# daigo0927/tf-raft

Hardware: NVIDIA B200
Metric: frame-pairs/sec at 448×512 iters=12; final-flow max-abs vs ref (higher is better)
Workload: dtype f32

## Files before the change

tf_raft_b200/csrc/conv_tc.cuh:

```cuda
#pragma once
#include <stdlib.h>

#include "common.cuh"
#include "tmap.cuh"

namespace raft {

enum TcEpilogue : int {
  EPI_LINEAR = 0,
  EPI_GRU_ZR = 1,
  EPI_GRU_Q = 2,
};
enum TcAct : int { ACT_NONE = 0, ACT_RELU = 1 };

constexpr int kEpiWarpsConv = 16;
constexpr int kTileM = 128;
constexpr int kChunkK = 64;
constexpr int kABytes = kTileM * kChunkK * 2;
constexpr int kEpiPatchBytes = 16 * 2048;
constexpr int kSmemBudget = 227 * 1024 - 2048;
constexpr int kARow3Pixels = 136;
constexpr int kARow3Bytes = 2 * kARow3Pixels * kChunkK * 2;

struct alignas(64) TcConvParams {
  CUtensorMap a_map[2];
  CUtensorMap b_map;
  int nseg, seg_chunks[2], seg_c0[2];
  int kh, kw, ph, pw;
  int stride;
  int B, H, W, TH, TW, tiles_x, tiles_y;
  int bn, n_total;
  int n_tiles_n;
  int nstages, stage_bytes, tmem_cols;
  int group_chunks;
  int mode, act;
  const float* bias;
  const float* inv_scale;
  float out_scale;
  float* out_f32; int f32_stride, f32_c0;
  __half* out_hi; __half* out_lo; int h_stride, h_c0;
  const float* post_scale;
  const float* post_shift;
  const float* residual; int res_stride, res_c0;
  const float* concat_src; int concat_n;
  float* z; int hid;
  float* h;
  long long* dbg;
  int pdl;
  int row3;
  float* adv_coords;
  float* adv_flow;
  int pair;
};

#if defined(__CUDA_ARCH__)
__device__ __forceinline__ float4 ld4(const float* p) { return *reinterpret_cast<const float4*>(p); }
__device__ __forceinline__ float4 ldg4(const float* p) { return __ldg(reinterpret_cast<const float4*>(p)); }
__device__ __forceinline__ void st4(float* p, float4 v) { *reinterpret_cast<float4*>(p) = v; }
__device__ __forceinline__ void st8u(void* p, const uint32_t (&r)[8]) {
#if defined(RAFT_EPI_EXP) && (RAFT_EPI_EXP & 1)
  if (r[0] != 0x7fc12345u) return;
#endif
  asm volatile("st.global.v8.b32 [%0], {%1, %2, %3, %4, %5, %6, %7, %8};" ::"l"(p), "r"(r[0]), "r"(r[1]), "r"(r[2]), "r"(r[3]),
               "r"(r[4]), "r"(r[5]), "r"(r[6]), "r"(r[7])
               : "memory");
}
__device__ __forceinline__ void ldcg8(const float* p, float (&r)[8]) {
#if defined(RAFT_EPI_EXP) && (RAFT_EPI_EXP & 2)
  if (p != nullptr) {
#pragma unroll
    for (int e = 0; e < 8; ++e) r[e] = 0.5f;
    return;
  }
#endif
  asm volatile("ld.global.cg.v8.f32 {%0, %1, %2, %3, %4, %5, %6, %7}, [%8];"
               : "=f"(r[0]), "=f"(r[1]), "=f"(r[2]), "=f"(r[3]), "=f"(r[4]), "=f"(r[5]), "=f"(r[6]), "=f"(r[7])
               : "l"(p));
}
__device__ __forceinline__ void ldnc8(const float* p, float (&r)[8]) {
  asm volatile("ld.global.nc.v8.f32 {%0, %1, %2, %3, %4, %5, %6, %7}, [%8];"
               : "=f"(r[0]), "=f"(r[1]), "=f"(r[2]), "=f"(r[3]), "=f"(r[4]), "=f"(r[5]), "=f"(r[6]), "=f"(r[7])
               : "l"(p));
}
__device__ __forceinline__ void st8f(float* p, float a, float b, float c, float d, float e, float f, float g, float h) {
  const uint32_t r[8] = {__float_as_uint(a), __float_as_uint(b), __float_as_uint(c), __float_as_uint(d),
                         __float_as_uint(e), __float_as_uint(f), __float_as_uint(g), __float_as_uint(h)};
  st8u(p, r);
}
__device__ __forceinline__ float4 ldcg4(const float* p) { return __ldcg(reinterpret_cast<const float4*>(p)); }

#if defined(RAFT_EPI_EXP) && (RAFT_EPI_EXP & 4)
__device__ __forceinline__ float fast_sigmoid(float x) { return x; }
#else
__device__ __forceinline__ float fast_sigmoid(float x) { return __fdividef(1.0f, 1.0f + __expf(-x)); }
#endif
__device__ __forceinline__ float fast_tanh(float x) { return 1.0f - __fdividef(2.0f, 1.0f + __expf(2.0f * x)); }

template <int MODE>
__device__ __forceinline__ void tc_epilogue_regs(const TcConvParams& p, float (&v)[32], size_t pix, int col, int ncol,
                                                 float inv_scale) {
  if (p.bias) {
#pragma unroll
    for (int q = 0; q < 8; ++q) {
      const float4 bq = ldg4(p.bias + col + 4 * q);
      v[4 * q] = v[4 * q] * inv_scale + bq.x; v[4 * q + 1] = v[4 * q + 1] * inv_scale + bq.y;
      v[4 * q + 2] = v[4 * q + 2] * inv_scale + bq.z; v[4 * q + 3] = v[4 * q + 3] * inv_scale + bq.w;
    }
  } else {
#pragma unroll
    for (int j = 0; j < 32; ++j) v[j] *= inv_scale;
  }
  if (MODE == EPI_LINEAR && p.post_scale) {
#pragma unroll
    for (int q = 0; q < 8; ++q) {
      const float4 sc = ldg4(p.post_scale + col + 4 * q), sh = ldg4(p.post_shift + col + 4 * q);
      v[4 * q] = v[4 * q] * sc.x + sh.x; v[4 * q + 1] = v[4 * q + 1] * sc.y + sh.y;
      v[4 * q + 2] = v[4 * q + 2] * sc.z + sh.z; v[4 * q + 3] = v[4 * q + 3] * sc.w + sh.w;
    }
  }

  __half* dhi = nullptr;
// ... 171 lines not shown
    for (int k = 0; k < 4; ++k)
#pragma unroll
      for (int e = 0; e < 4; ++e) v[k][e] *= inv_scale;
  }

  {
    const bool h_vec = ((p.h_stride | p.h_c0) & 3) == 0;
#pragma unroll
    for (int k0 = 0; k0 < 4; k0 += 2) {
      float4 zv[2], hv[2];
#pragma unroll
      for (int kk = 0; kk < 2; ++kk) {
        const bool ok = pixr[k0 + kk] >= 0;
        zv[kk] = ok ? ldcg4(p.z + (size_t)pixr[k0 + kk] * p.hid + col) : make_float4(0.f, 0.f, 0.f, 0.f);
        hv[kk] = ok ? ldcg4(p.h + (size_t)pixr[k0 + kk] * p.hid + col) : make_float4(0.f, 0.f, 0.f, 0.f);
      }
#pragma unroll
      for (int kk = 0; kk < 2; ++kk) {
        const int k = k0 + kk;
        if (pixr[k] < 0) continue;
        v[k][0] = (1.0f - zv[kk].x) * hv[kk].x + zv[kk].x * fast_tanh(v[k][0]);
        v[k][1] = (1.0f - zv[kk].y) * hv[kk].y + zv[kk].y * fast_tanh(v[k][1]);
        v[k][2] = (1.0f - zv[kk].z) * hv[kk].z + zv[kk].z * fast_tanh(v[k][2]);
        v[k][3] = (1.0f - zv[kk].w) * hv[kk].w + zv[kk].w * fast_tanh(v[k][3]);
        st4(p.h + (size_t)pixr[k] * p.hid + col, make_float4(v[k][0], v[k][1], v[k][2], v[k][3]));
        store_split4(p.out_hi, p.out_lo, (size_t)pixr[k] * p.h_stride + p.h_c0 + col, h_vec, v[k]);
      }
    }
  }
}

#endif

template <bool kRowEpi, bool kRow3 = false>
__global__ void __launch_bounds__(64 + 32 * kEpiWarpsConv, 1) conv_tc_kernel(const __grid_constant__ TcConvParams p) {
#if defined(__CUDA_ARCH__)
  constexpr int kEpiWarps = kEpiWarpsConv;
  extern __shared__ uint8_t smem_raw[];
  uint8_t* smem = reinterpret_cast<uint8_t*>((reinterpret_cast<uintptr_t>(smem_raw) + 1023) & ~uintptr_t(1023));
  const int nst = p.nstages;
  const int b_bytes = p.bn * kChunkK * 2;
  uint8_t* stages = smem;
  uint64_t* full_bar = reinterpret_cast<uint64_t*>(stages + (size_t)nst * p.stage_bytes);
  uint64_t* empty_bar = full_bar + nst;
  uint64_t* acc_full = empty_bar + nst;
  uint64_t* acc_empty = acc_full + 2;
  uint32_t* tmem_holder = reinterpret_cast<uint32_t*>(acc_empty + 2);
  float* patches = reinterpret_cast<float*>(stages + (size_t)nst * p.stage_bytes + 256);

  const int warp = threadIdx.x >> 5;
  const int lane = threadIdx.x & 31;

  const int mtiles = p.B * p.tiles_y * p.tiles_x;
  const int ntiles = mtiles * p.n_tiles_n;
  const int ntaps = p.kh * p.kw;
  const int chunks_per_tap = p.seg_chunks[0] + (p.nseg > 1 ? p.seg_chunks[1] : 0);
  const int total = (kRow3 ? p.kh : ntaps) * chunks_per_tap;
  const int gsz = p.group_chunks;
  const int ngroups = (total + gsz - 1) / gsz;
  const int nchunks32 = (p.bn + 31) >> 5;
  constexpr int kParts = kEpiWarps / 4;
  constexpr int kMaxCh = 8 / kParts;
  const int chunks_per_part = (nchunks32 + kParts - 1) / kParts;

  if (warp == 0 && lane == 0) {
    for (int s = 0; s < nst; ++s) {
      mbar_init(&full_bar[s], 1);
      mbar_init(&empty_bar[s], 1);
    }
    for (int i = 0; i < 2; ++i) {
      mbar_init(&acc_full[i], 1);
      mbar_init(&acc_empty[i], 4 * ((nchunks32 + chunks_per_part - 1) / chunks_per_part));
    }
    fence_mbar_init();
    prefetch_tmap(&p.a_map[0]);
    prefetch_tmap(&p.b_map);
    if (p.nseg > 1) prefetch_tmap(&p.a_map[1]);
  }
  if (warp == 1) {
    tmem_alloc(tmem_holder, (uint32_t)p.tmem_cols);
    tmem_relinquish();
  }
  tc_fence_before();
  __syncthreads();
  tc_fence_after();
  const uint32_t tmem_base = *tmem_holder;
  if (p.pdl && warp != 0) {
    asm volatile("griddepcontrol.wait;" ::: "memory");
    asm volatile("griddepcontrol.launch_dependents;" ::: "memory");
  }

  if (warp == 0) {
    if (elect_one()) {
      int it = 0;
      int npre = 0;
      if (p.pdl) {
        if (!kRow3 && (int)blockIdx.x < ntiles) {
          const int n0 = ((int)blockIdx.x / mtiles) * p.bn;
          npre = min(nst, total);
#pragma unroll 1
          for (int i = 0; i < npre; ++i) {
            mbar_arrive_expect_tx(&full_bar[i], (uint32_t)p.stage_bytes);
            tma_load_4d(stages + (size_t)i * p.stage_bytes + 2 * kABytes, &p.b_map, &full_bar[i], (i % chunks_per_tap) * kChunkK,
                        n0, i / chunks_per_tap, 0);
          }
        }
        asm volatile("griddepcontrol.wait;" ::: "memory");
        asm volatile("griddepcontrol.launch_dependents;" ::: "memory");
      }
      for (int t = blockIdx.x; t < ntiles; t += gridDim.x) {
        const int nt = t / mtiles;
        int mt = t - nt * mtiles;
        const int tx = mt % p.tiles_x;
        mt /= p.tiles_x;
        const int ty = mt % p.tiles_y;
        const int b = mt / p.tiles_y;
        const int x0 = tx * p.TW * p.stride, y0 = ty * p.TH * p.stride, n0 = nt * p.bn;
        if constexpr (kRow3) {
          for (int ky = 0; ky < p.kh; ++ky) {
            for (int ch = 0; ch < p.seg_chunks[0]; ++ch, ++it) {
              const int s = it % nst;
              mbar_wait(&empty_bar[s], ((uint32_t)(it / nst) & 1u) ^ 1u);
              if (p.dbg && blockIdx.x == 0 && it < 512) p.dbg[it] = clock64();
              uint8_t* st = stages + (size_t)s * p.stage_bytes;
              mbar_arrive_expect_tx(&full_bar[s], (uint32_t)p.stage_bytes);
              tma_load_5d(st, &p.a_map[0], &full_bar[s], p.seg_c0[0] + ch * kChunkK, x0 - p.pw, y0 + ky - p.ph, b, 0);
              tma_load_4d(st + kARow3Bytes, &p.b_map, &full_bar[s], ch * kChunkK, n0, ky * p.kw, 0);
            }
          }
        } else {
          for (int tap = 0; tap < ntaps; ++tap) {
            const int dy = tap / p.kw - p.ph, dx = tap % p.kw - p.pw;
            int kc = 0;
            for (int seg = 0; seg < p.nseg; ++seg) {
              for (int ch = 0; ch < p.seg_chunks[seg]; ++ch, ++kc, ++it) {
                const int s = it % nst;
                const uint32_t phase = (uint32_t)(it / nst) & 1u;
                mbar_wait(&empty_bar[s], phase ^ 1u);
                if (p.dbg && blockIdx.x == 0 && it < 512) p.dbg[it] = clock64();
                uint8_t* st = stages + (size_t)s * p.stage_bytes;
                const int c = p.seg_c0[seg] + ch * kChunkK;
#if defined(RAFT_TC_EXP) && (RAFT_TC_EXP & 6)
                if (RAFT_TC_EXP & 2) {
                  mbar_arrive_expect_tx(&full_bar[s], (uint32_t)(2 * kABytes));
                  tma_load_5d(st, &p.a_map[seg], &full_bar[s], c, x0 + dx, y0 + dy, b, 0);
                } else {
                  mbar_arrive_expect_tx(&full_bar[s], (uint32_t)(p.stage_bytes - 2 * kABytes));
                  tma_load_4d(st + 2 * kABytes, &p.b_map, &full_bar[s], kc * kChunkK, n0, tap, 0);
                }
#else
                if (it >= npre) mbar_arrive_expect_tx(&full_bar[s], (uint32_t)p.stage_bytes);
                tma_load_5d(st, &p.a_map[seg], &full_bar[s], c, x0 + dx, y0 + dy, b, 0);
                if (it >= npre) tma_load_4d(st + 2 * kABytes, &p.b_map, &full_bar[s], kc * kChunkK, n0, tap, 0);
#endif
              }
            }
          }
        }
      }
    }
  } else if (warp == 1) {
    const uint32_t idesc = make_idesc_f16(kTileM, p.bn);
    int it = 0, gg = 0;
    for (int t = blockIdx.x; t < ntiles; t += gridDim.x) {
      int done = 0;
      for (int g = 0; g < ngroups; ++g, ++gg) {
        const int buf = gg & 1;
        mbar_wait(&acc_empty[buf], ((uint32_t)(gg >> 1) & 1u) ^ 1u);
        tc_fence_after();
        if (p.dbg && blockIdx.x == 0 && gg < 256 && lane == 0) p.dbg[1024 + 256 + gg] = clock64();
        const uint32_t d_tmem = tmem_base + (uint32_t)(buf * p.bn);
        const int gend = min(total, done + gsz);
        for (int first = 1; done < gend; ++done, ++it, first = 0) {
          const int s = it % nst;
          const uint32_t phase = (uint32_t)(it / nst) & 1u;
          mbar_wait(&full_bar[s], phase);
          tc_fence_after();
          if (p.dbg && blockIdx.x == 0 && it < 512 && lane == 0) p.dbg[512 + it] = clock64();
          if (elect_one()) {
            const uint32_t sa = smem_u32(stages + (size_t)s * p.stage_bytes);
            if constexpr (kRow3) {
#pragma unroll 1
              for (int dx = 0; dx < 3; ++dx) {
                const uint64_t a_hi = make_desc_sw128(sa + dx * 128);
                const uint64_t a_lo = make_desc_sw128(sa + kARow3Bytes / 2 + dx * 128);
                const uint64_t b_hi = make_desc_sw128(sa + kARow3Bytes + dx * b_bytes);
                const uint64_t b_lo = make_desc_sw128(sa + kARow3Bytes + (3 + dx) * b_bytes);
                umma_chunk3<false>(d_tmem, a_hi, a_lo, b_hi, b_lo, idesc, first != 0 && dx == 0);
              }
            } else {
              const uint64_t a_hi = make_desc_sw128(sa);
              const uint64_t a_lo = make_desc_sw128(sa + kABytes);
              const uint64_t b_hi = make_desc_sw128(sa + 2 * kABytes);
              const uint64_t b_lo = make_desc_sw128(sa + 2 * kABytes + b_bytes);
#if defined(RAFT_TC_EXP) && (RAFT_TC_EXP & 1)
              if (sa != 0xffffffffu) goto tc_exp_skip_mma;
#endif
              umma_chunk3<false>(d_tmem, a_hi, a_lo, b_hi, b_lo, idesc, first != 0);
#if defined(RAFT_TC_EXP) && (RAFT_TC_EXP & 1)
            tc_exp_skip_mma:;
#endif
            }
            umma_commit(&empty_bar[s]);
            if (done == gend - 1) umma_commit(&acc_full[buf]);
          }
          __syncwarp();
        }
      }
    }
  } else {
    const int quarter = warp & 3;
    const int part_id = (warp - 2) >> 2;
    const int chunk0 = part_id * chunks_per_part;
    const int my_chunks = max(0, min(chunks_per_part, nchunks32 - chunk0));
    const int m = quarter * 32 + lane;
    const int xl = m % p.TW, yl = m / p.TW;
    const float inv_scale = p.inv_scale ? __ldg(p.inv_scale) : 1.0f;
    const uint32_t trow = tmem_base + ((uint32_t)(quarter * 32) << 16);

    if (my_chunks > 0) {
      int gg = 0;
      for (int t = blockIdx.x; t < ntiles; t += gridDim.x) {
        float racc[kMaxCh][32];
#pragma unroll
        for (int ci = 0; ci < kMaxCh; ++ci)
#pragma unroll
          for (int j = 0; j < 32; ++j) racc[ci][j] = 0.0f;

        for (int g = 0; g < ngroups; ++g, ++gg) {
          const int buf = gg & 1;
          mbar_wait(&acc_full[buf], (uint32_t)(gg >> 1) & 1u);
          tc_fence_after();
          if (p.dbg && blockIdx.x == 0 && gg < 256 && warp == 2 && lane == 0) p.dbg[1024 + gg] = clock64();
#pragma unroll
          for (int ci = 0; ci < kMaxCh; ++ci) {
            if (ci < my_chunks) {
              const int c0 = (chunk0 + ci) * 32;
              uint32_t r[32];
              if (p.bn - c0 >= 32) {
                tmem_ld_32x32(trow + (uint32_t)(buf * p.bn + c0), r);
              } else {
                uint32_t r16[16];
// ... 103 lines not shown
  p.tiles_y = ceil_div(p.H, p.TH);
  p.stage_bytes = 2 * kABytes + 2 * (p.pair ? p.bn / 2 : p.bn) * kChunkK * 2;
  if (p.row3) p.stage_bytes = kARow3Bytes + 3 * 2 * p.bn * kChunkK * 2;
  const int patch = tc_uses_patch(p.mode) ? kEpiPatchBytes : 0;
  int nst = (kSmemBudget - patch) / p.stage_bytes;
  if (nst > 8) nst = 8;
  p.nstages = nst;
  int cols = 32;
  while (cols < 2 * p.bn) cols <<= 1;
  p.tmem_cols = cols;
  if (p.group_chunks <= 0) p.group_chunks = 2;
  return nst * p.stage_bytes + 1024  + 256  + patch;
}

inline bool tc_pdl_enabled() {
  static const int pdl = [] { const char* e = getenv("RAFT_B200_PDL"); return e ? atoi(e) : 1; }();
  return pdl != 0;
}

inline int tc_launch(TcConvParams& p, int n_tiles_n, cudaStream_t stream) {
  if (p.bn % 16 != 0 || p.bn < 16 || p.bn > 256 || p.TW * p.TH != kTileM) return RAFT_ERR_BAD_SHAPE;
  if (p.mode != EPI_LINEAR && p.mode != EPI_GRU_ZR && p.mode != EPI_GRU_Q) return RAFT_ERR_UNSUPPORTED;
  if (p.stride < 1) p.stride = 1;
  const int smem = tc_finalize(p);
  if (p.nstages < 2) return RAFT_ERR_UNSUPPORTED;
  int dev = 0;
  RAFT_CUDA_TRY(cudaGetDevice(&dev));
  const unsigned long long dev_bit = 1ull << (dev & 63);
  static unsigned long long attr_set_mask = 0;
  if (!(attr_set_mask & dev_bit)) {
    RAFT_CUDA_TRY(cudaFuncSetAttribute(conv_tc_kernel<false>, cudaFuncAttributeMaxDynamicSharedMemorySize, 227 * 1024));
    RAFT_CUDA_TRY(cudaFuncSetAttribute(conv_tc_kernel<true>, cudaFuncAttributeMaxDynamicSharedMemorySize, 227 * 1024));
    RAFT_CUDA_TRY(cudaFuncSetAttribute(conv_tc_kernel<true, true>, cudaFuncAttributeMaxDynamicSharedMemorySize, 227 * 1024));
    attr_set_mask |= dev_bit;
  }
  const int mtiles = p.B * p.tiles_y * p.tiles_x;
  p.n_tiles_n = n_tiles_n;
  const long ntiles = (long)mtiles * n_tiles_n;
  const unsigned grid = (unsigned)(ntiles < kNumSMs ? ntiles : kNumSMs);
  p.pdl = tc_pdl_enabled() ? 1 : 0;
  const int threads = 64 + 32 * kEpiWarpsConv;
  if (p.row3 && (p.mode != EPI_LINEAR || p.kh != 3 || p.kw != 3 || p.stride != 1 || p.TH != 1 || p.TW != kTileM || p.nseg != 1 ||
                 p.bn % 8 != 0 || n_tiles_n != 1))
    return RAFT_ERR_UNSUPPORTED;
  void (*kern)(TcConvParams) = p.mode == EPI_GRU_Q ? conv_tc_kernel<false> : (p.row3 ? conv_tc_kernel<true, true> : conv_tc_kernel<true>);
  if (!p.pdl) {
    kern<<<grid, threads, smem, stream>>>(p);
  } else {
    cudaLaunchConfig_t cfg;
    memset(&cfg, 0, sizeof(cfg));
    cfg.gridDim = dim3(grid);
    cfg.blockDim = dim3((unsigned)threads);
    cfg.dynamicSmemBytes = (size_t)smem;
    cfg.stream = stream;
    cudaLaunchAttribute attr[1];
    attr[0].id = cudaLaunchAttributeProgrammaticStreamSerialization;
    attr[0].val.programmaticStreamSerializationAllowed = 1;
    cfg.attrs = attr;
    cfg.numAttrs = 1;
    RAFT_CUDA_TRY(cudaLaunchKernelEx(&cfg, kern, p));
  }
  return raft_launch_status();
}

}
```

tf_raft_b200/csrc/encoder.cuh:

```cuda
#pragma once
#include <algorithm>

#include "lookup.cuh"
#include "update.cuh"

namespace raft {

enum { NORM_NONE = 0, NORM_INSTANCE = 1, NORM_BATCH = 2 };

struct EncSpec { int c0; int c[3]; int s[3]; };
inline EncSpec enc_spec(int variant) {
  if (variant == RAFT_VARIANT_BASIC) return {64, {64, 96, 128}, {1, 2, 2}};
  return {32, {32, 64, 96}, {1, 2, 2}};
}
inline int pad64(int c) { return round_up(c, 64); }

struct EncConvSlot { size_t hi, lo, bias, scale, absmax; int kh, kw, cin, cout, cin_pad, cout_pad; };
struct EncNormSlot { size_t gamma, beta, fscale, fshift; int C; };
struct EncLayout {
  EncConvSlot conv1;
  EncNormSlot norm1;
  EncConvSlot bc1[6], bc2[6], bds[6];
  EncNormSlot bn1[6], bn2[6], bnd[6];
  int has_ds[6], bcin[6], bc[6], bstride[6];
// ... 20 lines not shown
  auto norm_slot = [&](int C) {
    EncNormSlot n;
    n.C = C;
    n.gamma = take(sizeof(float) * (C + 64)); n.beta = take(sizeof(float) * (C + 64));
    n.fscale = take(sizeof(float) * (C + 64)); n.fshift = take(sizeof(float) * (C + 64));
    return n;
  };
  L.conv1 = conv_slot(1, 1, 147, S.c0);
  L.norm1 = norm_slot(S.c0);
  int cin = S.c0;
  for (int k = 0; k < 6; ++k) {
    const int c = S.c[k / 2], st = (k % 2 == 0) ? S.s[k / 2] : 1;
    L.bcin[k] = cin; L.bc[k] = c; L.bstride[k] = st;
    L.bc1[k] = conv_slot(3, 3, cin, c);
    L.bc2[k] = conv_slot(3, 3, c, c);
    L.bn1[k] = norm_slot(c);
    L.bn2[k] = norm_slot(c);
    L.has_ds[k] = st != 1;
    if (L.has_ds[k]) { L.bds[k] = conv_slot(1, 1, cin, c); L.bnd[k] = norm_slot(c); }
    cin = c;
  }
  L.conv2 = conv_slot(1, 1, cin, out_dim);
  L.total = off;
  return L;
}

struct EncWs {
  float *X32, *O32, *Y32, *D32;
  __half *Xh, *Xl, *Oh, *Ol, *Fh, *Fl, *Ih, *Il;
  float *part, *mean, *mult;
  size_t total;
};
constexpr int kNormSplit = 64;
inline EncWs enc_ws_layout(void* base, int variant, int N, int H, int W) {
  EncWs E;
  memset(&E, 0, sizeof(E));
  const EncSpec S = enc_spec(variant);
  size_t max32 = 0, max16 = 0;
  for (int l = 0; l < 3; ++l) {
    const int d = 2 << l;
    const size_t np = (size_t)N * ((H + d - 1) / d) * ((W + d - 1) / d);
    const int c = l == 0 ? (S.c0 > S.c[0] ? S.c0 : S.c[0]) : S.c[l];
    if (np * c > max32) max32 = np * c;
    if (np * pad64(c) > max16) max16 = np * pad64(c);
  }
  uint8_t* b8 = reinterpret_cast<uint8_t*>(base);
  size_t off = 0;
  auto take = [&](size_t bytes) { uint8_t* p = b8 + off; off = align_up(off + bytes, 1024); return p; };
  E.X32 = (float*)take(max32 * 4); E.O32 = (float*)take(max32 * 4);
  E.Y32 = (float*)take(max32 * 4); E.D32 = (float*)take(max32 * 4);
  E.Xh = (__half*)take(max16 * 2); E.Xl = (__half*)take(max16 * 2);
  E.Oh = (__half*)take(max16 * 2); E.Ol = (__half*)take(max16 * 2);
  E.Fh = (__half*)take(max16 * 2); E.Fl = (__half*)take(max16 * 2);
  {
    const size_t np1 = (size_t)N * ((H + 1) / 2) * ((W + 1) / 2);
    E.Ih = (__half*)take(np1 * 192 * 2); E.Il = (__half*)take(np1 * 192 * 2);
  }
  E.part = (float*)take((size_t)N * kNormSplit * 3 * 256 * 4);
  E.mean = (float*)take((size_t)N * 256 * 4);
  E.mult = (float*)take((size_t)N * 256 * 4);
  E.total = off;
  return E;
}

inline int enc_pack_conv(const raft_conv& cv, const EncConvSlot& s, uint8_t* base, cudaStream_t st) {
  if (!cv.kernel || !cv.bias) return RAFT_ERR_BAD_ARG;
  if (cv.kh != s.kh || cv.kw != s.kw || cv.cin != s.cin || cv.cout != s.cout) return RAFT_ERR_BAD_SHAPE;
  const size_t nw = (size_t)s.kh * s.kw * s.cin * s.cout;
  unsigned int* amax = reinterpret_cast<unsigned int*>(base + s.absmax);
  float* scale = reinterpret_cast<float*>(base + s.scale);
  absmax_kernel<<<grid_for(nw), 256, 0, st>>>(cv.kernel, nw, amax);
  weight_scale_kernel<<<1, 1, 0, st>>>(amax, scale);
  PackParams pp;
  memset(&pp, 0, sizeof(pp));
  pp.w = cv.kernel; pp.kh = s.kh; pp.kw = s.kw; pp.cin = s.cin; pp.cout = s.cout;
  pp.hi = reinterpret_cast<__half*>(base + s.hi); pp.lo = reinterpret_cast<__half*>(base + s.lo);
  pp.cout_pad = s.cout_pad; pp.cin_pad = s.cin_pad; pp.cout_off = 0;
  pp.nrange = 1; pp.r_src0[0] = 0; pp.r_n[0] = s.cin; pp.r_dst0[0] = 0;
  pp.scale = scale;
  pack_weights_kernel<<<grid_for(nw), 256, 0, st>>>(pp);
  g_launches += 3;
  RAFT_CUDA_TRY(cudaMemcpyAsync(base + s.bias, cv.bias, s.cout * sizeof(float), cudaMemcpyDeviceToDevice, st));
  return raft_launch_status();
}

inline int enc_pack_norm(const raft_norm& nm, const EncNormSlot& s, int norm_type, uint8_t* base, cudaStream_t st) {
  if (norm_type == NORM_NONE) return 0;
  if (!nm.gamma || !nm.beta) return RAFT_ERR_BAD_ARG;
  float* g = reinterpret_cast<float*>(base + s.gamma);
// ... 30 lines not shown
    RAFT_TRY(enc_pack_conv(w->block[k].conv2, L.bc2[k], base, st));
    RAFT_TRY(enc_pack_norm(w->block[k].norm1, L.bn1[k], norm_type, base, st));
    RAFT_TRY(enc_pack_norm(w->block[k].norm2, L.bn2[k], norm_type, base, st));
    if (L.has_ds[k]) {
      RAFT_TRY(enc_pack_conv(w->block[k].downsample, L.bds[k], base, st));
      RAFT_TRY(enc_pack_norm(w->block[k].downsample_norm, L.bnd[k], norm_type, base, st));
    }
  }
  RAFT_TRY(enc_pack_conv(w->conv2, L.conv2, base, st));
  return raft_launch_status();
}

struct EncCtx {
  const uint8_t* prep; EncLayout L; EncWs W; cudaStream_t st;
  int N, norm_type, stats;
  int per_image;
};

inline int enc_norm_apply(const EncCtx& c, const EncNormSlot& ns, const float* y, size_t npix, int P, int relu,
                          const float* skip32, const __half* skip_hi, const __half* skip_lo, float* out32, __half* hi,
                          __half* lo) {
  const int C = ns.C, G = c.per_image ? c.N : 1;
  const int Pg = c.per_image ? P : (int)npix;
  const float* gamma = reinterpret_cast<const float*>(c.prep + ns.gamma);
  const float* beta = reinterpret_cast<const float*>(c.prep + ns.beta);
  norm_stats_kernel<<<dim3((unsigned)G, kNormSplit), 256, 0, c.st>>>(y, Pg, C, kNormSplit, c.W.part);
  norm_final_kernel<<<ceil_div(G * C * 32, 256), 256, 0, c.st>>>(c.W.part, G, C, kNormSplit, gamma, 1e-3f, c.W.mean, c.W.mult);
  norm_apply_kernel<<<grid_for(npix * (pad64(C) / 8)), 256, 0, c.st>>>(y, npix, P, C, c.per_image, c.W.mean, c.W.mult, beta, relu,
                                                                 skip32, skip_hi, skip_lo, out32, hi, lo, pad64(C));
  g_launches += 3;
  return raft_launch_status();
}

inline int enc_conv_tc(const EncCtx& c, const EncConvSlot& cs, const EncNormSlot* ns, const __half* ahi, const __half* alo,
                       int Hin, int Win, int Hout, int Wout, int stride, int relu, const float* skip, float* out32,
                       __half* ohi, __half* olo) {
  TcConvParams p;
  memset(&p, 0, sizeof(p));
  int tw, th;
  tc_pick_tile(Wout, Hout, &tw, &th);
  if (tw * stride > 256) tw = 128 / stride, th = 128 / tw;
  static const int row3_flag = [] { const char* e = getenv("RAFT_B200_ROW3"); return e ? atoi(e) : 1; }();
  const bool row3 = row3_flag && cs.kh == 3 && cs.kw == 3 && stride == 1 && tw == kTileM && th == 1 && cs.cout_pad <= 96 &&
                    cs.cout_pad % 8 == 0;
  if (row3) {
    RAFT_TRY(make_tmap_act2(&p.a_map[0], ahi, alo, c.N, Hin, Win, cs.cin_pad, kARow3Pixels, 1, 1));
    RAFT_TRY(make_tmap_wgt3(&p.b_map, reinterpret_cast<const __half*>(c.prep + cs.hi),
                            reinterpret_cast<const __half*>(c.prep + cs.lo), cs.kh * cs.kw, cs.cout_pad, cs.cin_pad, cs.cout_pad));
    p.row3 = 1;
  } else {
    RAFT_TRY(make_tmap_act2(&p.a_map[0], ahi, alo, c.N, Hin, Win, cs.cin_pad, tw, th, stride));
    RAFT_TRY(make_tmap_wgt2(&p.b_map, reinterpret_cast<const __half*>(c.prep + cs.hi),
                            reinterpret_cast<const __half*>(c.prep + cs.lo), cs.kh * cs.kw, cs.cout_pad, cs.cin_pad,
                            cs.cout_pad));
  }
  p.nseg = 1; p.seg_chunks[0] = cs.cin_pad / kChunkK; p.seg_c0[0] = 0;
  p.kh = cs.kh; p.kw = cs.kw; p.stride = stride;
  if (stride == 1) { p.ph = (cs.kh - 1) / 2; p.pw = (cs.kw - 1) / 2; }
  else {
    const int tot_h = (Hout - 1) * stride + cs.kh - Hin, tot_w = (Wout - 1) * stride + cs.kw - Win;
    p.ph = (tot_h > 0 ? tot_h : 0) / 2; p.pw = (tot_w > 0 ? tot_w : 0) / 2;
  }
  p.B = c.N; p.H = Hout; p.W = Wout; p.TH = th; p.TW = tw;
  p.bn = cs.cout_pad; p.n_total = cs.cout;
  p.mode = EPI_LINEAR; p.out_scale = 1.0f;
  p.bias = reinterpret_cast<const float*>(c.prep + cs.bias);
  p.inv_scale = reinterpret_cast<const float*>(c.prep + cs.scale) + 1;
  p.out_f32 = out32; p.f32_stride = cs.cout; p.f32_c0 = 0;
  p.out_hi = ohi; p.out_lo = olo; p.h_stride = pad64(cs.cout); p.h_c0 = 0;
  if (ns && !c.stats && c.norm_type == NORM_BATCH) {
    p.post_scale = reinterpret_cast<const float*>(c.prep + ns->fscale);
    p.post_shift = reinterpret_cast<const float*>(c.prep + ns->fshift);
  }
  const bool fused = !(ns && c.stats);
  if (fused) {
    p.act = relu ? ACT_RELU : ACT_NONE;
    p.residual = skip; p.res_stride = cs.cout; p.res_c0 = 0;
  } else {
    p.act = ACT_NONE; p.out_hi = nullptr; p.out_lo = nullptr;
  }
  if (g_dbg_layer >= 1000 && g_dbg_count++ == g_dbg_layer - 1000) p.dbg = g_dbg_buf;
  {
    static const int grp = [] { const char* e = getenv("RAFT_B200_ENC_GROUP"); return e ? atoi(e) : 5; }();
    if (grp > 0) p.group_chunks = grp;
    if (row3) p.group_chunks = 2;
  }
  ++g_launches;
  return tc_launch(p, 1, c.st);
}

inline int encoder_forward(int variant, int norm_type, int out_dim, const void* prepared, const float* images, int N,
                           int H, int W, int training, int image_norm, float* out, void* ws, size_t ws_bytes, cudaStream_t st) {
  EncCtx c;
  c.prep = reinterpret_cast<const uint8_t*>(prepared);
  c.L = enc_layout(variant, out_dim);
  c.W = enc_ws_layout(ws, variant, N, H, W);
  if (c.W.total > ws_bytes) return RAFT_ERR_WORKSPACE;
  c.st = st; c.N = N; c.norm_type = norm_type;
  c.stats = (norm_type == NORM_INSTANCE) || (norm_type == NORM_BATCH && training);
  c.per_image = norm_type == NORM_INSTANCE;
  const EncSpec S = enc_spec(variant);
  const EncLayout& L = c.L;
  const EncWs& E = c.W;

  int h = (H + 1) / 2, w = (W + 1) / 2;
  {
    const size_t npix = (size_t)N * h * w;
    const int tot_h = (h - 1) * 2 + 7 - H, tot_w = (w - 1) * 2 + 7 - W;
    const float* src = images;
    if (image_norm) {
      const size_t nimg = (size_t)N * H * W * 3;
      image_norm_kernel<<<grid_for(nimg), 256, 0, st>>>(images, E.O32, nimg);
      ++g_launches;
      src = E.O32;
    }
    stem_im2col_kernel<<<grid_for(npix * 24), 256, 0, st>>>(src, N, H, W, h, w, (tot_h > 0 ? tot_h : 0) / 2,
                                                            (tot_w > 0 ? tot_w : 0) / 2, 0, E.Ih, E.Il);
    ++g_launches;
    if (!c.stats && pad64(S.c0) != S.c0) {
      RAFT_CUDA_TRY(cudaMemsetAsync(E.Xh, 0, npix * pad64(S.c0) * 2, st));
      RAFT_CUDA_TRY(cudaMemsetAsync(E.Xl, 0, npix * pad64(S.c0) * 2, st));
    }
    RAFT_TRY(enc_conv_tc(c, L.conv1, &L.norm1, E.Ih, E.Il, h, w, h, w, 1, 1, nullptr, c.stats ? E.Y32 : E.X32, E.Xh, E.Xl));
    if (c.stats) RAFT_TRY(enc_norm_apply(c, L.norm1, E.Y32, npix, h * w, 1, nullptr, nullptr, nullptr, nullptr, E.Xh, E.Xl));
  }

  float *X32 = E.X32, *O32 = E.O32;
  __half *Xh = E.Xh, *Xl = E.Xl, *Oh = E.Oh, *Ol = E.Ol;
  for (int k = 0; k < 6; ++k) {
    const int st2 = L.bstride[k], cin = L.bcin[k], cc = L.bc[k];
    const int ho = (h + st2 - 1) / st2, wo = (w + st2 - 1) / st2;
    const size_t npo = (size_t)N * ho * wo;
    (void)cin;
    const bool zero_pad_out = pad64(cc) != cc;
    if (!c.stats && zero_pad_out) {
      RAFT_CUDA_TRY(cudaMemsetAsync(E.Fh, 0, npo * pad64(cc) * 2, st));
      RAFT_CUDA_TRY(cudaMemsetAsync(E.Fl, 0, npo * pad64(cc) * 2, st));
      RAFT_CUDA_TRY(cudaMemsetAsync(Oh, 0, npo * pad64(cc) * 2, st));
      RAFT_CUDA_TRY(cudaMemsetAsync(Ol, 0, npo * pad64(cc) * 2, st));
    }
    RAFT_TRY(enc_conv_tc(c, L.bc1[k], &L.bn1[k], Xh, Xl, h, w, ho, wo, st2, 1, nullptr, c.stats ? E.Y32 : nullptr, E.Fh, E.Fl));
    if (c.stats) RAFT_TRY(enc_norm_apply(c, L.bn1[k], E.Y32, npo, ho * wo, 1, nullptr, nullptr, nullptr, nullptr, E.Fh, E.Fl));
    const float* skip = X32;
    if (L.has_ds[k]) {
      RAFT_TRY(enc_conv_tc(c, L.bds[k], &L.bnd[k], Xh, Xl, h, w, ho, wo, st2, 0, nullptr, c.stats ? E.Y32 : E.D32, nullptr, nullptr));
      if (c.stats) RAFT_TRY(enc_norm_apply(c, L.bnd[k], E.Y32, npo, ho * wo, 0, nullptr, nullptr, nullptr, E.D32, nullptr, nullptr));
      skip = E.D32;
    }
    RAFT_TRY(enc_conv_tc(c, L.bc2[k], &L.bn2[k], E.Fh, E.Fl, ho, wo, ho, wo, 1, 1, skip, c.stats ? E.Y32 : O32, Oh, Ol));
    if (c.stats) {
      if (L.has_ds[k]) RAFT_TRY(enc_norm_apply(c, L.bn2[k], E.Y32, npo, ho * wo, 1, E.D32, nullptr, nullptr, nullptr, Oh, Ol));
      else RAFT_TRY(enc_norm_apply(c, L.bn2[k], E.Y32, npo, ho * wo, 1, nullptr, Xh, Xl, nullptr, Oh, Ol));
    }
    float* t32 = X32; X32 = O32; O32 = t32;
    __half* th_ = Xh; Xh = Oh; Oh = th_;
    __half* tl_ = Xl; Xl = Ol; Ol = tl_;
// ... 8 lines not shown
```

tf_raft_b200/csrc/kernels.cuh:

```cuda
#pragma once
#include "common.cuh"

namespace raft {

__global__ void split_plane_kernel(const float* __restrict__ src, int src_stride, int src_c0, int nch, int nch_pad,
                                   __half* __restrict__ hi, __half* __restrict__ lo, int dst_stride, int dst_c0,
                                   size_t npix, float scale) {
  const size_t total = npix * (size_t)nch_pad;
  for (size_t i = blockIdx.x * (size_t)blockDim.x + threadIdx.x; i < total; i += (size_t)gridDim.x * blockDim.x) {
    const size_t px = i / nch_pad;
    const int c = (int)(i - px * nch_pad);
    __half h = __float2half_rn(0.f), l = h;
    if (c < nch) split_f16(src[px * src_stride + src_c0 + c] * scale, h, l);
    hi[px * dst_stride + dst_c0 + c] = h;
    lo[px * dst_stride + dst_c0 + c] = l;
  }
}

__global__ void avgpool2x2_kernel(const float* __restrict__ src, float* __restrict__ dst, size_t M, int H, int W,
                                  int C) {
  const int Ho = H / 2, Wo = W / 2;
  const size_t total = M * (size_t)Ho * Wo * C;
  for (size_t i = blockIdx.x * (size_t)blockDim.x + threadIdx.x; i < total; i += (size_t)gridDim.x * blockDim.x) {
    size_t t = i;
// ... 531 lines not shown
        const float ss[8] = {s0.x, s0.y, s0.z, s0.w, s1.x, s1.y, s1.z, s1.w};
#pragma unroll
        for (int e = 0; e < 8; ++e) v[e] = fmaxf(ss[e] + v[e], 0.f);
      } else if (skip_hi) {
        const uint4 h4 = *reinterpret_cast<const uint4*>(skip_hi + px * c_pad + c), l4 = *reinterpret_cast<const uint4*>(skip_lo + px * c_pad + c);
        const uint32_t hw[4] = {h4.x, h4.y, h4.z, h4.w}, lw[4] = {l4.x, l4.y, l4.z, l4.w};
#pragma unroll
        for (int e = 0; e < 4; ++e) {
          const float2 hf = __half22float2(*reinterpret_cast<const __half2*>(&hw[e]));
          const float2 lf = __half22float2(*reinterpret_cast<const __half2*>(&lw[e]));
          v[2 * e] = fmaxf(hf.x + lf.x + v[2 * e], 0.f);
          v[2 * e + 1] = fmaxf(hf.y + lf.y + v[2 * e + 1], 0.f);
        }
      }
      if (out32) {
        *reinterpret_cast<float4*>(out32 + px * C + c) = make_float4(v[0], v[1], v[2], v[3]);
        *reinterpret_cast<float4*>(out32 + px * C + c + 4) = make_float4(v[4], v[5], v[6], v[7]);
      }
    }
    if (hi) {
      uint32_t ph[4], pl[4];
#pragma unroll
      for (int e = 0; e < 4; ++e) split_f16x2(v[2 * e], v[2 * e + 1], ph[e], pl[e]);
      *reinterpret_cast<uint4*>(hi + px * c_pad + c) = make_uint4(ph[0], ph[1], ph[2], ph[3]);
      *reinterpret_cast<uint4*>(lo + px * c_pad + c) = make_uint4(pl[0], pl[1], pl[2], pl[3]);
    }
  }
}
__global__ void image_norm_kernel(const float* __restrict__ img, float* __restrict__ out, size_t n) {
  for (size_t i = blockIdx.x * (size_t)blockDim.x + threadIdx.x; i < n; i += (size_t)gridDim.x * blockDim.x)
    out[i] = __fsub_rn(__fmul_rn(2.0f, __fdiv_rn(img[i], 255.0f)), 1.0f);
}

__global__ void stem_im2col_kernel(const float* __restrict__ img, int N, int H, int W, int h, int w, int pad_t,
                                   int pad_l, int image_norm, __half* __restrict__ hi, __half* __restrict__ lo) {
  const size_t total = (size_t)N * h * w * 24;
  for (size_t i = blockIdx.x * (size_t)blockDim.x + threadIdx.x; i < total; i += (size_t)gridDim.x * blockDim.x) {
    const int grp = (int)(i % 24);
    const size_t px = i / 24;
    const int x = (int)(px % w), y = (int)((px / w) % h), n = (int)(px / ((size_t)w * h));
    uint32_t ph[4] = {0u, 0u, 0u, 0u}, pl[4] = {0u, 0u, 0u, 0u};
    if (grp * 8 < 147) {
      int ty = (grp * 8) / 21, j = grp * 8 - ty * 21;
      const int ix0 = 2 * x - pad_l;
      const float* base = img + ((size_t)n * H * W + ix0) * 3;
      float v[8];
#pragma unroll
      for (int e = 0; e < 8; ++e) {
        const int iy = 2 * y + ty - pad_t, ix = ix0 + ((j * 11) >> 5);
        v[e] = 0.f;
        if (ty < 7 && iy >= 0 && iy < H && ix >= 0 && ix < W) {
          v[e] = __ldg(base + (ptrdiff_t)iy * W * 3 + j);
          if (image_norm) v[e] = __fsub_rn(__fmul_rn(2.0f, __fdiv_rn(v[e], 255.0f)), 1.0f);
        }
        if (++j == 21) { j = 0; ++ty; }
      }
#pragma unroll
      for (int e = 0; e < 4; ++e) split_f16x2(v[2 * e], v[2 * e + 1], ph[e], pl[e]);
    }
    reinterpret_cast<uint4*>(hi)[i] = make_uint4(ph[0], ph[1], ph[2], ph[3]);
    reinterpret_cast<uint4*>(lo)[i] = make_uint4(pl[0], pl[1], pl[2], pl[3]);
  }
}

__device__ __forceinline__ void flow_im2col_rider(const float* __restrict__ flow, int B, int h, int w, __half* __restrict__ hi,
                                                  __half* __restrict__ lo, size_t tid, size_t nthreads) {
  const size_t total = (size_t)B * h * w * 16;
  for (size_t i = tid; i < total; i += nthreads) {
    const int g = (int)(i & 15);
    const size_t px = i >> 4;
    const int x = (int)(px % w), y = (int)((px / w) % h);
    uint32_t ph[4], pl[4];
#pragma unroll
    for (int e = 0; e < 4; ++e) {
      const int tap = 4 * g + e;
      float2 v = make_float2(0.f, 0.f);
      if (tap < 49) {
        const int yy = y + tap / 7 - 3, xx = x + tap % 7 - 3;
        if (yy >= 0 && yy < h && xx >= 0 && xx < w)
          v = __ldg(reinterpret_cast<const float2*>(flow) + (ptrdiff_t)px + (ptrdiff_t)(yy - y) * w + (xx - x));
      }
      split_f16x2(v.x, v.y, ph[e], pl[e]);
    }
    reinterpret_cast<uint4*>(hi)[i] = make_uint4(ph[0], ph[1], ph[2], ph[3]);
    reinterpret_cast<uint4*>(lo)[i] = make_uint4(pl[0], pl[1], pl[2], pl[3]);
  }
}

__global__ void flow_im2col_kernel(const float* __restrict__ flow, int B, int h, int w, __half* __restrict__ hi,
                                   __half* __restrict__ lo) {
  const size_t total = (size_t)B * h * w * 128;
  for (size_t i = blockIdx.x * (size_t)blockDim.x + threadIdx.x; i < total; i += (size_t)gridDim.x * blockDim.x) {
// ... 47 lines not shown
```

Baseline: 555.2.

## Fuse stem im2col into tensor-core conv via in-kernel gather warps

Adds a gather mode to the tcgen05 conv kernel. Half of the epilogue warps build the 7x7 stride-2 stem im2col A tiles directly in shared memory, with the swizzle and hi/lo fp16 split, and signal the full barrier, while TMA loads only the weights. This removes the separate stem_im2col kernel launch and its large hi/lo global buffer round trip. In exchange the kernel has fewer epilogue warps free for output, and the register-heavy gather may stall the MMA pipeline.

```diff
diff --git a/tf_raft_b200/csrc/conv_tc.cuh b/tf_raft_b200/csrc/conv_tc.cuh
--- a/tf_raft_b200/csrc/conv_tc.cuh
+++ b/tf_raft_b200/csrc/conv_tc.cuh
@@ -2,6 +2,7 @@
 #include <stdlib.h>
 
 #include "common.cuh"
+#include "kernels.cuh"
 #include "tmap.cuh"
 
 namespace raft {
@@ -21,6 +22,8 @@
 constexpr int kSmemBudget = 227 * 1024 - 2048;
 constexpr int kARow3Pixels = 136;
 constexpr int kARow3Bytes = 2 * kARow3Pixels * kChunkK * 2;
+constexpr int kGatherWarps = kEpiWarpsConv / 2;
+constexpr int kGatherWarp0 = 2 + kEpiWarpsConv - kGatherWarps;
 
 struct alignas(64) TcConvParams {
   CUtensorMap a_map[2];
@@ -51,6 +54,8 @@
   float* adv_coords;
   float* adv_flow;
   int pair;
+  int gather;
+  const float* gather_img; int gather_H, gather_W, gather_pad_t, gather_pad_l;
 };
 
 #if defined(__CUDA_ARCH__)
@@ -87,6 +92,9 @@
                          __float_as_uint(e), __float_as_uint(f), __float_as_uint(g), __float_as_uint(h)};
   st8u(p, r);
 }
+__device__ __forceinline__ void sts128(uint32_t addr, const uint32_t (&r)[4]) {
+  asm volatile("st.shared.v4.b32 [%0], {%1, %2, %3, %4};" ::"r"(addr), "r"(r[0]), "r"(r[1]), "r"(r[2]), "r"(r[3]) : "memory");
+}
 __device__ __forceinline__ float4 ldcg4(const float* p) { return __ldcg(reinterpret_cast<const float4*>(p)); }
 
 #if defined(RAFT_EPI_EXP) && (RAFT_EPI_EXP & 4)
@@ -324,7 +332,7 @@
 
 #endif
 
-template <bool kRowEpi, bool kRow3 = false>
+template <bool kRowEpi, bool kRow3 = false, bool kGather = false>
 __global__ void __launch_bounds__(64 + 32 * kEpiWarpsConv, 1) conv_tc_kernel(const __grid_constant__ TcConvParams p) {
 #if defined(__CUDA_ARCH__)
   constexpr int kEpiWarps = kEpiWarpsConv;
@@ -355,9 +363,10 @@
   constexpr int kMaxCh = 8 / kParts;
   const int chunks_per_part = (nchunks32 + kParts - 1) / kParts;
 
+  const uint32_t tx_bytes = (uint32_t)(kGather ? p.stage_bytes - 2 * kABytes : p.stage_bytes);
   if (warp == 0 && lane == 0) {
     for (int s = 0; s < nst; ++s) {
-      mbar_init(&full_bar[s], 1);
+      mbar_init(&full_bar[s], kGather ? 1 + kGatherWarps : 1);
       mbar_init(&empty_bar[s], 1);
     }
     for (int i = 0; i < 2; ++i) {
@@ -365,7 +374,7 @@
       mbar_init(&acc_empty[i], 4 * ((nchunks32 + chunks_per_part - 1) / chunks_per_part));
     }
     fence_mbar_init();
-    prefetch_tmap(&p.a_map[0]);
+    if (!kGather) prefetch_tmap(&p.a_map[0]);
     prefetch_tmap(&p.b_map);
     if (p.nseg > 1) prefetch_tmap(&p.a_map[1]);
   }
@@ -392,7 +401,7 @@
           npre = min(nst, total);
 #pragma unroll 1
           for (int i = 0; i < npre; ++i) {
-            mbar_arrive_expect_tx(&full_bar[i], (uint32_t)p.stage_bytes);
+            mbar_arrive_expect_tx(&full_bar[i], tx_bytes);
             tma_load_4d(stages + (size_t)i * p.stage_bytes + 2 * kABytes, &p.b_map, &full_bar[i], (i % chunks_per_tap) * kChunkK,
                         n0, i / chunks_per_tap, 0);
           }
@@ -441,8 +450,8 @@
                   tma_load_4d(st + 2 * kABytes, &p.b_map, &full_bar[s], kc * kChunkK, n0, tap, 0);
                 }
 #else
-                if (it >= npre) mbar_arrive_expect_tx(&full_bar[s], (uint32_t)p.stage_bytes);
-                tma_load_5d(st, &p.a_map[seg], &full_bar[s], c, x0 + dx, y0 + dy, b, 0);
+                if (it >= npre) mbar_arrive_expect_tx(&full_bar[s], tx_bytes);
+                if (!kGather) tma_load_5d(st, &p.a_map[seg], &full_bar[s], c, x0 + dx, y0 + dy, b, 0);
                 if (it >= npre) tma_load_4d(st + 2 * kABytes, &p.b_map, &full_bar[s], kc * kChunkK, n0, tap, 0);
 #endif
               }
@@ -500,6 +509,57 @@
         }
       }
     }
+  } else if (kGather && warp >= kGatherWarp0) {
+    constexpr int kUnits = 8 * kTileM / (32 * kGatherWarps);
+    constexpr int kStemChunks = kStemKPad / kChunkK;
+    const int gt = (int)threadIdx.x - 32 * kGatherWarp0;
+    const int m = gt & (kTileM - 1);
+    const bool upper = gt >= kTileM;
+    const int xl = m % p.TW, yl = m / p.TW;
+    int it = 0;
+    for (int t = blockIdx.x; t < ntiles; t += gridDim.x) {
+      int mt = t % mtiles;
+      const int tx = mt % p.tiles_x;
+      mt /= p.tiles_x;
+      const int ty = mt % p.tiles_y;
+      const int b = mt / p.tiles_y;
+      const int x = tx * p.TW + xl, y = ty * p.TH + yl;
+      const bool inside = x < p.W && y < p.H;
+#pragma unroll
+      for (int ch = 0; ch < kStemChunks; ++ch, ++it) {
+        const int s = it % nst;
+        float v[kUnits][8];
+#pragma unroll
+        for (int k = 0; k < kUnits; ++k)
+#pragma unroll
+          for (int e = 0; e < 8; ++e) v[k][e] = 0.f;
+        if (inside) {
+          if (upper) {
+#pragma unroll
+            for (int k = 0; k < kUnits; ++k)
+              stem_window8(p.gather_img, p.gather_H, p.gather_W, p.gather_pad_t, p.gather_pad_l, 0, b, y, x, ch * 8 + kUnits + k, v[k]);
+          } else {
+#pragma unroll
+            for (int k = 0; k < kUnits; ++k)
+              stem_window8(p.gather_img, p.gather_H, p.gather_W, p.gather_pad_t, p.gather_pad_l, 0, b, y, x, ch * 8 + k, v[k]);
+          }
+        }
+        mbar_wait(&empty_bar[s], ((uint32_t)(it / nst) & 1u) ^ 1u);
+        const uint32_t sa = smem_u32(stages + (size_t)s * p.stage_bytes) + (uint32_t)(m * 128);
+#pragma unroll
+        for (int k = 0; k < kUnits; ++k) {
+          uint32_t ph[4], pl[4];
+#pragma unroll
+          for (int e = 0; e < 4; ++e) split_f16x2(v[k][2 * e], v[k][2 * e + 1], ph[e], pl[e]);
+          const uint32_t off = (uint32_t)((((upper ? kUnits : 0) + k) ^ (m & 7)) << 4);
+          sts128(sa + off, ph);
+          sts128(sa + kABytes + off, pl);
+        }
+        fence_proxy_async();
+        __syncwarp();
+        if (lane == 0) mbar_arrive(&full_bar[s]);
+      }
+    }
   } else {
     const int quarter = warp & 3;
     const int part_id = (warp - 2) >> 2;
@@ -669,6 +729,7 @@
     RAFT_CUDA_TRY(cudaFuncSetAttribute(conv_tc_kernel<false>, cudaFuncAttributeMaxDynamicSharedMemorySize, 227 * 1024));
     RAFT_CUDA_TRY(cudaFuncSetAttribute(conv_tc_kernel<true>, cudaFuncAttributeMaxDynamicSharedMemorySize, 227 * 1024));
     RAFT_CUDA_TRY(cudaFuncSetAttribute(conv_tc_kernel<true, true>, cudaFuncAttributeMaxDynamicSharedMemorySize, 227 * 1024));
+    RAFT_CUDA_TRY(cudaFuncSetAttribute(conv_tc_kernel<true, false, true>, cudaFuncAttributeMaxDynamicSharedMemorySize, 227 * 1024));
     attr_set_mask |= dev_bit;
   }
   const int mtiles = p.B * p.tiles_y * p.tiles_x;
@@ -680,7 +741,13 @@
   if (p.row3 && (p.mode != EPI_LINEAR || p.kh != 3 || p.kw != 3 || p.stride != 1 || p.TH != 1 || p.TW != kTileM || p.nseg != 1 ||
                  p.bn % 8 != 0 || n_tiles_n != 1))
     return RAFT_ERR_UNSUPPORTED;
-  void (*kern)(TcConvParams) = p.mode == EPI_GRU_Q ? conv_tc_kernel<false> : (p.row3 ? conv_tc_kernel<true, true> : conv_tc_kernel<true>);
+  if (p.gather && (p.mode != EPI_LINEAR || p.kh != 1 || p.kw != 1 || p.stride != 1 || p.row3 || p.nseg != 1 || p.seg_c0[0] != 0 ||
+                   p.seg_chunks[0] * kChunkK != kStemKPad || p.bn > 64 || n_tiles_n != 1 || !p.gather_img))
+    return RAFT_ERR_UNSUPPORTED;
+  void (*kern)(TcConvParams) = p.mode == EPI_GRU_Q ? conv_tc_kernel<false>
+                               : p.row3            ? conv_tc_kernel<true, true>
+                               : p.gather          ? conv_tc_kernel<true, false, true>
+                                                   : conv_tc_kernel<true>;
   if (!p.pdl) {
     kern<<<grid, threads, smem, stream>>>(p);
   } else {
diff --git a/tf_raft_b200/csrc/encoder.cuh b/tf_raft_b200/csrc/encoder.cuh
--- a/tf_raft_b200/csrc/encoder.cuh
+++ b/tf_raft_b200/csrc/encoder.cuh
@@ -76,6 +76,12 @@
   size_t total;
 };
 constexpr int kNormSplit = 64;
+
+inline bool stem_gather_enabled() {
+  static const int v = [] { const char* e = getenv("RAFT_B200_STEM_GATHER"); return e ? atoi(e) : 1; }();
+  return v != 0;
+}
+
 inline EncWs enc_ws_layout(void* base, int variant, int N, int H, int W) {
   EncWs E;
   memset(&E, 0, sizeof(E));
@@ -96,9 +102,9 @@
   E.Xh = (__half*)take(max16 * 2); E.Xl = (__half*)take(max16 * 2);
   E.Oh = (__half*)take(max16 * 2); E.Ol = (__half*)take(max16 * 2);
   E.Fh = (__half*)take(max16 * 2); E.Fl = (__half*)take(max16 * 2);
-  {
+  if (!stem_gather_enabled()) {
     const size_t np1 = (size_t)N * ((H + 1) / 2) * ((W + 1) / 2);
-    E.Ih = (__half*)take(np1 * 192 * 2); E.Il = (__half*)take(np1 * 192 * 2);
+    E.Ih = (__half*)take(np1 * kStemKPad * 2); E.Il = (__half*)take(np1 * kStemKPad * 2);
   }
   E.part = (float*)take((size_t)N * kNormSplit * 3 * 256 * 4);
   E.mean = (float*)take((size_t)N * 256 * 4);
@@ -195,9 +201,11 @@
   return raft_launch_status();
 }
 
+struct StemGather { const float* img; int H, W, pad_t, pad_l; };
+
 inline int enc_conv_tc(const EncCtx& c, const EncConvSlot& cs, const EncNormSlot* ns, const __half* ahi, const __half* alo,
                        int Hin, int Win, int Hout, int Wout, int stride, int relu, const float* skip, float* out32,
-                       __half* ohi, __half* olo) {
+                       __half* ohi, __half* olo, const StemGather* gather = nullptr) {
   TcConvParams p;
   memset(&p, 0, sizeof(p));
   int tw, th;
@@ -206,7 +214,14 @@
   static const int row3_flag = [] { const char* e = getenv("RAFT_B200_ROW3"); return e ? atoi(e) : 1; }();
   const bool row3 = row3_flag && cs.kh == 3 && cs.kw == 3 && stride == 1 && tw == kTileM && th == 1 && cs.cout_pad <= 96 &&
                     cs.cout_pad % 8 == 0;
-  if (row3) {
+  if (gather) {
+    RAFT_TRY(make_tmap_wgt2(&p.b_map, reinterpret_cast<const __half*>(c.prep + cs.hi),
+                            reinterpret_cast<const __half*>(c.prep + cs.lo), cs.kh * cs.kw, cs.cout_pad, cs.cin_pad,
+                            cs.cout_pad));
+    p.gather = 1;
+    p.gather_img = gather->img; p.gather_H = gather->H; p.gather_W = gather->W;
+    p.gather_pad_t = gather->pad_t; p.gather_pad_l = gather->pad_l;
+  } else if (row3) {
     RAFT_TRY(make_tmap_act2(&p.a_map[0], ahi, alo, c.N, Hin, Win, cs.cin_pad, kARow3Pixels, 1, 1));
     RAFT_TRY(make_tmap_wgt3(&p.b_map, reinterpret_cast<const __half*>(c.prep + cs.hi),
                             reinterpret_cast<const __half*>(c.prep + cs.lo), cs.kh * cs.kw, cs.cout_pad, cs.cin_pad, cs.cout_pad));
@@ -270,6 +285,7 @@
   {
     const size_t npix = (size_t)N * h * w;
     const int tot_h = (h - 1) * 2 + 7 - H, tot_w = (w - 1) * 2 + 7 - W;
+    const int pad_t = (tot_h > 0 ? tot_h : 0) / 2, pad_l = (tot_w > 0 ? tot_w : 0) / 2;
     const float* src = images;
     if (image_norm) {
       const size_t nimg = (size_t)N * H * W * 3;
@@ -277,14 +293,18 @@
       ++g_launches;
       src = E.O32;
     }
-    stem_im2col_kernel<<<grid_for(npix * 24), 256, 0, st>>>(src, N, H, W, h, w, (tot_h > 0 ? tot_h : 0) / 2,
-                                                            (tot_w > 0 ? tot_w : 0) / 2, 0, E.Ih, E.Il);
-    ++g_launches;
+    const bool gather = stem_gather_enabled();
+    if (!gather) {
+      stem_im2col_kernel<<<grid_for(npix * (kStemKPad / 8)), 256, 0, st>>>(src, N, H, W, h, w, pad_t, pad_l, 0, E.Ih, E.Il);
+      ++g_launches;
+    }
     if (!c.stats && pad64(S.c0) != S.c0) {
       RAFT_CUDA_TRY(cudaMemsetAsync(E.Xh, 0, npix * pad64(S.c0) * 2, st));
       RAFT_CUDA_TRY(cudaMemsetAsync(E.Xl, 0, npix * pad64(S.c0) * 2, st));
     }
-    RAFT_TRY(enc_conv_tc(c, L.conv1, &L.norm1, E.Ih, E.Il, h, w, h, w, 1, 1, nullptr, c.stats ? E.Y32 : E.X32, E.Xh, E.Xl));
+    const StemGather sg = {src, H, W, pad_t, pad_l};
+    RAFT_TRY(enc_conv_tc(c, L.conv1, &L.norm1, E.Ih, E.Il, h, w, h, w, 1, 1, nullptr, c.stats ? E.Y32 : E.X32, E.Xh, E.Xl,
+                         gather ? &sg : nullptr));
     if (c.stats) RAFT_TRY(enc_norm_apply(c, L.norm1, E.Y32, npix, h * w, 1, nullptr, nullptr, nullptr, nullptr, E.Xh, E.Xl));
   }
 
diff --git a/tf_raft_b200/csrc/kernels.cuh b/tf_raft_b200/csrc/kernels.cuh
--- a/tf_raft_b200/csrc/kernels.cuh
+++ b/tf_raft_b200/csrc/kernels.cuh
@@ -587,32 +587,40 @@
     out[i] = __fsub_rn(__fmul_rn(2.0f, __fdiv_rn(img[i], 255.0f)), 1.0f);
 }
 
+constexpr int kStemK = 147;
+constexpr int kStemKPad = 192;
+
+__device__ __forceinline__ void stem_window8(const float* __restrict__ img, int H, int W, int pad_t, int pad_l, int image_norm,
+                                             int n, int y, int x, int grp, float (&v)[8]) {
+#pragma unroll
+  for (int e = 0; e < 8; ++e) v[e] = 0.f;
+  if (grp * 8 >= kStemK) return;
+  int ty = (grp * 8) / 21, j = grp * 8 - ty * 21;
+  const int ix0 = 2 * x - pad_l;
+  const float* base = img + ((size_t)n * H * W + ix0) * 3;
+#pragma unroll
+  for (int e = 0; e < 8; ++e) {
+    const int iy = 2 * y + ty - pad_t, ix = ix0 + ((j * 11) >> 5);
+    if (ty < 7 && iy >= 0 && iy < H && ix >= 0 && ix < W) {
+      v[e] = __ldg(base + (ptrdiff_t)iy * W * 3 + j);
+      if (image_norm) v[e] = __fsub_rn(__fmul_rn(2.0f, __fdiv_rn(v[e], 255.0f)), 1.0f);
+    }
+    if (++j == 21) { j = 0; ++ty; }
+  }
+}
+
 __global__ void stem_im2col_kernel(const float* __restrict__ img, int N, int H, int W, int h, int w, int pad_t,
                                    int pad_l, int image_norm, __half* __restrict__ hi, __half* __restrict__ lo) {
-  const size_t total = (size_t)N * h * w * 24;
-  for (size_t i = blockIdx.x * (size_t)blockDim.x + threadIdx.x; i < total; i += (size_t)gridDim.x * blockDim.x) {
-    const int grp = (int)(i % 24);
-    const size_t px = i / 24;
+  const size_t total = (size_t)N * h * w * (kStemKPad / 8);
+  for (size_t i = blockIdx.x * (size_t)blockDim.x + threadIdx.x; i < total; i += (size_t)gridDim.x * blockDim.x) {
+    const int grp = (int)(i % (kStemKPad / 8));
+    const size_t px = i / (kStemKPad / 8);
     const int x = (int)(px % w), y = (int)((px / w) % h), n = (int)(px / ((size_t)w * h));
-    uint32_t ph[4] = {0u, 0u, 0u, 0u}, pl[4] = {0u, 0u, 0u, 0u};
-    if (grp * 8 < 147) {
-      int ty = (grp * 8) / 21, j = grp * 8 - ty * 21;
-      const int ix0 = 2 * x - pad_l;
-      const float* base = img + ((size_t)n * H * W + ix0) * 3;
-      float v[8];
-#pragma unroll
-      for (int e = 0; e < 8; ++e) {
-        const int iy = 2 * y + ty - pad_t, ix = ix0 + ((j * 11) >> 5);
-        v[e] = 0.f;
-        if (ty < 7 && iy >= 0 && iy < H && ix >= 0 && ix < W) {
-          v[e] = __ldg(base + (ptrdiff_t)iy * W * 3 + j);
-          if (image_norm) v[e] = __fsub_rn(__fmul_rn(2.0f, __fdiv_rn(v[e], 255.0f)), 1.0f);
-        }
-        if (++j == 21) { j = 0; ++ty; }
-      }
-#pragma unroll
-      for (int e = 0; e < 4; ++e) split_f16x2(v[2 * e], v[2 * e + 1], ph[e], pl[e]);
-    }
+    float v[8];
+    stem_window8(img, H, W, pad_t, pad_l, image_norm, n, y, x, grp, v);
+    uint32_t ph[4], pl[4];
+#pragma unroll
+    for (int e = 0; e < 4; ++e) split_f16x2(v[2 * e], v[2 * e + 1], ph[e], pl[e]);
     reinterpret_cast<uint4*>(hi)[i] = make_uint4(ph[0], ph[1], ph[2], ph[3]);
     reinterpret_cast<uint4*>(lo)[i] = make_uint4(pl[0], pl[1], pl[2], pl[3]);
   }
```

New measurement: 565.1 (median of 6 runs). +1.8%, better.
